# myfavouritekk/vdetlib

Hardware: AMD Instinct MI355X
Metric: boxes/sec whole-node (NMS+temporal-conv+link), 300f×10k-box synth; mAP parity (higher is better)
Workload: dtype f32; 1 GPU; configs[1]+[2]: 1 video/GPU, 300 frames x 10000 boxes x 200 classes; per-(frame,class) NMS thresh 0.30 + temporal max-pool w=3 + 3-tap temporal convolution; greedy tubelets: 10 tracks/class (stop < 0.90), IoU-link >= 0.50, spatial max-pool IoU > 0.70 + completion + temporal max-pool; frames=300, boxes=10000, classes=200, scores=rand, parallelism=video-per-gpu x1, 4 distinct videos in flight per GPU

## Files before the change

### vdetlib_amd/csrc/nms_kernels.hpp

```cpp
#pragma once
#include <hip/hip_runtime.h>
#include <stdint.h>

namespace vdet {

struct GroupDesc {
    int32_t box_off;
    int32_t nbox;
    int64_t bits_off;
};

__device__ __host__ __forceinline__ int64_t bit_word(int nbox, int v, int c)
{
    const int W = (nbox + 63) >> 6;
    return ((int64_t)(v >> 6) * W + c) * 64 + (v & 63);
}
__host__ __device__ __forceinline__ int64_t bit_words_of_group(int nbox)
{
    const int64_t W = (nbox + 63) >> 6;
    return W * W * 64;
}

struct TileDesc {
    int32_t group;
// ... 1034 lines not shown
        const uint32_t cnt = (uint32_t)__popcll(peers);
        if (act && (r1 != rank || r2 != cnt + rank)) nbad = 1;
        __builtin_amdgcn_fence(__ATOMIC_ACQ_REL, "wavefront");
    }
    if (__ballot(nbad) && lane == 0) atomicOr(bad, 1);
}

__global__ __launch_bounds__(256) void transpose_keys_kernel(const float *__restrict__ scores, uint32_t *__restrict__ keys,
                                                             int B, int C, int use_thr, float thr)
{
    __shared__ uint32_t tile[64][65];
    const int f = blockIdx.z;
    const int b0 = blockIdx.x * 64, c0 = blockIdx.y * 64;
    const int tx = threadIdx.x & 63, ty = threadIdx.x >> 6;
    const float *src = scores + (int64_t)f * B * C;
    for (int r = ty; r < 64; r += 4) {
        const int b = b0 + r, c = c0 + tx;
        uint32_t k = 0;
        if (b < B && c < C) {
            const float s = src[(int64_t)b * C + c];
            k = score_key(s);
            if (use_thr && !(s > thr)) k = 0u;
        }
        tile[r][tx] = k;
    }
    __syncthreads();
    uint32_t *dst = keys + (int64_t)f * C * B;
    for (int r = ty; r < 64; r += 4) {
        const int c = c0 + r, b = b0 + tx;
        if (c < C && b < B) dst[(int64_t)c * B + b] = tile[tx][r];
    }
}

struct WalkParams {
    int mode, P, B, C;
    const GroupDesc *groups;
    const uint16_t *order;
    const int32_t *ncand;
    const uint2 *row_meta;
    const uint16_t *adj;
    const uint32_t *group_z;
    int32_t *keep_idx;
    int32_t *keep_cnt;
    int64_t cap;
    int *status;
    int mask_words;
    const uint32_t *group_flags;
    int wave_words;
    int packed;
    const WalkMeta *wmeta;
    float t32;
    int adj32;
    const uint4 *wmeta16;
};

typedef __attribute__((address_space(3))) uint32_t lds_u32_t;
typedef volatile lds_u32_t *lds_mask_t;

__device__ __forceinline__ lds_mask_t lds_mask_ptr(unsigned char *dyn_smem, int word_off)
{
    return (lds_mask_t)((__attribute__((address_space(3))) unsigned char *)dyn_smem) + word_off;
}
__device__ __forceinline__ void lds_or(lds_mask_t m, int word, uint32_t bits)
{
    __hip_atomic_fetch_or((lds_u32_t *)(m + word), bits, __ATOMIC_RELAXED, __HIP_MEMORY_SCOPE_WAVEFRONT);
}
__device__ __forceinline__ void lds_and(lds_mask_t m, int word, uint32_t bits)
{
    __hip_atomic_fetch_and((lds_u32_t *)(m + word), bits, __ATOMIC_RELAXED, __HIP_MEMORY_SCOPE_WAVEFRONT);
}

__device__ __forceinline__ void lds_or_pair(lds_mask_t m, uint32_t d)
{
    uint32_t w0, w1;
    asm("v_bfe_u32 %0, %1, 5, 11" : "=v"(w0) : "v"(d));
    asm("v_bfe_u32 %0, %1, 21, 11" : "=v"(w1) : "v"(d));
    lds_or(m, (int)w0, 1u << (d & 31u));
    lds_or(m, (int)w1, 1u << ((d >> 16) & 31u));
}

constexpr int kWalkGrp = 4;

template <bool HASZ>
__device__ __forceinline__ void walk_apply_slice(lds_mask_t mask, uint16_t e, bool in_range, int &bad)
{
    if (HASZ) {
        if (in_range) {
            const int v = e & 0x7FFF;
            if (e & kZTag) { if (!((mask[v >> 5] >> (v & 31)) & 1u)) bad = 1; }
            else lds_or(mask, v >> 5, 1u << (v & 31));
        }
    } else {
        if (in_range) lds_or(mask, e >> 5, 1u << (e & 31));
    }
}

template <bool HASZ>
__device__ __forceinline__ void walk_group(lds_mask_t mask, const uint16_t *__restrict__ adj, int lane, int c,
                                           uint32_t off, int deg, const int (&ls)[kWalkGrp], int ng,
                                           const uint32_t (&pre)[kWalkGrp], unsigned long long &kept_lanes, int &bad)
{
#pragma unroll
    for (int k = 0; k < kWalkGrp; ++k) {
        if (k >= ng) break;
        const int cu = __builtin_amdgcn_readlane(c, ls[k]);
        if (__builtin_amdgcn_readfirstlane((mask[cu >> 5] >> (cu & 31)) & 1u)) continue;
// ... 56 lines not shown
        if (surv_s) {
            const int pos = nk + (int)__builtin_amdgcn_mbcnt_hi((uint32_t)(surv_s >> 32),
                                                               __builtin_amdgcn_mbcnt_lo((uint32_t)surv_s, 0u));
            if (surv && sub == 0 && (int64_t)pos < cap) out[(uint32_t)pos] = cm;
            nk += __popcll(surv_s);
            const uint32_t off = surv ? __float_as_uint(mi.y) : 0u;
            const int deg = surv ? (int)__float_as_uint(mi.z) : 0;
            AdjVec a0, a1;
            if (prm.adj32) {
                const uint32_t bo = off * 2u;
                const char *ab = reinterpret_cast<const char *>(prm.adj);
                a0 = *reinterpret_cast<const AdjVec *>(ab + (bo + (8 * sub < deg ? 16u * (uint32_t)sub : 0u)));
                a1 = *reinterpret_cast<const AdjVec *>(ab + (bo + (64 + 8 * sub < deg ? 128u + 16u * (uint32_t)sub : 0u)));
            } else {
                const AdjVec *pa = reinterpret_cast<const AdjVec *>(prm.adj + off);
                a0 = pa[8 * sub < deg ? sub : 0];
                a1 = pa[64 + 8 * sub < deg ? 8 + sub : 0];
            }
            const bool has0 = 8 * sub < deg, has1 = 64 + 8 * sub < deg;
            if (has0) {
#pragma unroll
                for (int t = 0; t < 4; ++t) {
                    const uint32_t d = a0.v[t];
                    lds_or_pair(mask, d);
                }
            }
            if (__ballot(has1) != 0ull) {
                if (has1) {
#pragma unroll
                    for (int t = 0; t < 4; ++t) {
                        const uint32_t d = a1.v[t];
                        lds_or_pair(mask, d);
                    }
                }
                unsigned long long lg = __ballot(sub == 0 && deg > 128);
                while (lg) {
                    const int l = __ffsll((unsigned long long)lg) - 1;
                    lg &= lg - 1;
                    const uint32_t o = __builtin_amdgcn_readlane(off, l);
                    const int dl = __builtin_amdgcn_readlane(deg, l);
                    for (int e0 = 128; e0 < dl; e0 += 64) {
                        const uint32_t e = prm.adj[o + min(e0 + lane, dl - 1)];
                        if (e0 + lane < dl) lds_or(mask, (int)(e >> 5), 1u << (e & 31u));
                    }
                }
            }
            __builtin_amdgcn_s_waitcnt(0x0F70);
        }
        qh = ring_wrap(qh + ng);
        qn -= ng;
    }
}

template <bool U16>
__device__ __forceinline__ void walk_list_packed(const WalkParams &prm, lds_mask_t mask, const int lane, const int rb,
                                                 const uint16_t *__restrict__ order, const int ncand,
                                                 int32_t *__restrict__ out, const int64_t cap, int &nk_out)
{
    lds_mask_t ring = mask + prm.mask_words;
    lds_f4_t ringb = (lds_f4_t)ring;
    const WalkMeta *__restrict__ wmeta = prm.wmeta + rb;
    const uint4 *__restrict__ wm16 = U16 ? prm.wmeta16 + rb : nullptr;
    const float t32 = prm.t32;
    int qh = 0, qn = 0, nk = 0;
    const int last = max(ncand - 1, 0);
    int cc[3];
    uint2 mm[3];
    float4 bb[3];
    uint4 rr[3];
    cc[0] = (int)order[(uint32_t)min(lane, last)];
    cc[1] = (int)order[(uint32_t)min(64 + lane, last)];
    cc[2] = 0;
    mm[0] = mm[1] = mm[2] = make_uint2(0u, 0u);
    bb[0] = bb[1] = bb[2] = make_float4(0.f, 0.f, 0.f, 0.f);
    rr[0] = rr[1] = rr[2] = make_uint4(0u, 0u, 0u, 0u);
    if (lane < ncand) {
        if (U16) rr[0] = wm16[(uint32_t)cc[0]];
        else { const WalkMeta *wm = wmeta + (uint32_t)cc[0]; bb[0] = wm->box; const uint4 rw = wm->row; mm[0] = make_uint2(rw.x, rw.y); }
    }
#define VDET_WALK_PASS(Q0, CUR, NXT, NN)                                                                                             \
    {                                                                                                                                \
        const int q0_ = (Q0);                                                                                                        \
        const int c = cc[CUR];                                                                                                       \
        cc[NN] = (int)order[(uint32_t)min(q0_ + 128 + lane, last)];                                                                  \
        {    \
             \
            const bool want = (q0_ + 64 + lane) < ncand && !((mask[cc[NXT] >> 5] >> (cc[NXT] & 31)) & 1u);                           \
            if (U16) rr[NXT] = wm16[want ? (uint32_t)cc[NXT] : 0u];                                                                  \
            else {                                                                                                                   \
                const WalkMeta *wm = wmeta + (want ? (uint32_t)cc[NXT] : 0u);                                                        \
                bb[NXT] = wm->box; const uint4 rw = wm->row; mm[NXT] = make_uint2(rw.x, rw.y);                                       \
            }                                                                                                                        \
        }                                                                                                                            \
        const bool alive = (q0_ + lane) < ncand && !((mask[c >> 5] >> (c & 31)) & 1u);                                               \
        const unsigned long long am = __ballot(alive);                                                                               \
        if (alive) {                                                                                                                 \
            const int s = ring_wrap(qh + qn + (int)__builtin_amdgcn_mbcnt_hi((uint32_t)(am >> 32), __builtin_amdgcn_mbcnt_lo((uint32_t)am, 0u))); \
            ring[8 * s] = (uint32_t)c;                                                                                               \
            lds_f4v bv;                                                                                                              \
            if (U16) {                                                                                                               \
                ring[8 * s + 1] = rr[CUR].z;                                                                                         \
                ring[8 * s + 2] = rr[CUR].w;                                                                                         \
                bv.x = (float)(rr[CUR].x & 0xFFFFu); bv.y = (float)(rr[CUR].x >> 16);                                                \
                bv.z = (float)(rr[CUR].y & 0xFFFFu); bv.w = (float)(rr[CUR].y >> 16);                                                \
            } else {                                                                                                                 \
                ring[8 * s + 1] = mm[CUR].x;                                                                                         \
                ring[8 * s + 2] = mm[CUR].y;                                                                                         \
                bv.x = bb[CUR].x; bv.y = bb[CUR].y; bv.z = bb[CUR].z; bv.w = bb[CUR].w;                                              \
            }                                                                                                                        \
            ringb[2 * s + 1] = bv;                                                                                                   \
            ring[8 * s + 3] = __float_as_uint(box_area(make_float4(bv.x, bv.y, bv.z, bv.w)));                                        \
        }                                                                                                                            \
        qn += __popcll(am);                                                                                                          \
        walk_ring_drain(prm, mask, ring, ringb, lane, t32, q0_ + 64 >= ncand, qh, qn, nk, out, cap);                                 \
    }
    for (int q0 = 0; q0 < ncand; q0 += 192) {
        VDET_WALK_PASS(q0, 0, 1, 2)
        if (q0 + 64 >= ncand) break;
        VDET_WALK_PASS(q0 + 64, 1, 2, 0)
        if (q0 + 128 >= ncand) break;
        VDET_WALK_PASS(q0 + 128, 2, 0, 1)
    }
#undef VDET_WALK_PASS
    nk_out = nk;
}

__device__ __forceinline__ void walk_one(const WalkParams &prm, const int p, unsigned char *smem, const int lane, const int w)
{
    lds_mask_t mask = lds_mask_ptr(smem, w * prm.wave_words);
    const ProblemRef pr = decode_problem(prm.mode, p, prm.B, prm.C, prm.groups);
    const int N = pr.N, rb = pr.rb;
    const uint16_t *order = prm.order + pr.obase;
    const int ncand = prm.ncand[p];
    const bool has_z = prm.group_z[pr.g] != 0;
    const bool regular = !has_z && prm.group_flags && (prm.group_flags[pr.g] & kFlagRegular);
    int32_t *out = prm.keep_idx + (prm.mode == 2 ? (int64_t)rb : (int64_t)p * prm.cap);
    const int64_t cap = prm.mode == 2 ? (int64_t)N : prm.cap;

    for (int i = lane; i < ((N + 31) >> 5); i += 64) mask[i] = 0u;
    __builtin_amdgcn_fence(__ATOMIC_ACQ_REL, "wavefront");
    if (has_z) {
        for (int q = ncand + lane; q < N; q += 64) {
            const int v = order[q];
            lds_or(mask, v >> 5, 1u << (v & 31));
        }
        __builtin_amdgcn_fence(__ATOMIC_ACQ_REL, "wavefront");
    }

    int nk = 0;
    int bad = 0;
    if (regular && prm.packed && N >= 2) {
        if (prm.wmeta16 && (prm.group_flags[pr.g] & kFlagU16)) walk_list_packed<true>(prm, mask, lane, rb, order, ncand, out, cap, nk);
        else walk_list_packed<false>(prm, mask, lane, rb, order, ncand, out, cap, nk);
        if (lane == 0) prm.keep_cnt[p] = nk;
        if ((int64_t)nk > cap && lane == 0) atomicOr(prm.status, kStCap);
        return;
    }
    const uint32_t *adjw = reinterpret_cast<const uint32_t *>(prm.adj);
    const int last = max(ncand - 1, 0);
    int c_cur = (int)order[min(lane, last)];
    int c_nxt = (int)order[min(64 + lane, last)];
    uint2 m_cur = make_uint2(0u, 0u);
    if (lane < ncand) m_cur = prm.row_meta[rb + c_cur];
    for (int q0 = 0; q0 < ncand; q0 += 64) {
        const int q = q0 + lane;
        const bool valid = q < ncand;
        const int c = c_cur;
        const int c_nn = (int)order[min(q0 + 128 + lane, last)];
        uint2 m_nxt = make_uint2(0u, 0u);
        if ((q + 64) < ncand && !((mask[c_nxt >> 5] >> (c_nxt & 31)) & 1u)) m_nxt = prm.row_meta[rb + c_nxt];
        const bool alive = valid && !((mask[c >> 5] >> (c & 31)) & 1u);
        unsigned long long am = __ballot(alive);
        unsigned long long kept_lanes = 0ull;
        const uint32_t off = m_cur.x;
        const int deg = (int)m_cur.y;
        while (am) {
            int ls[kWalkGrp];
            int ng = 0;
#pragma unroll
            for (int k = 0; k < kWalkGrp; ++k) {
                ls[k] = k ? ls[k - 1] : 0;
                if (am) { ls[k] = __builtin_amdgcn_readfirstlane(__ffsll((unsigned long long)am) - 1); am &= am - 1; ng = k + 1; }
            }
            uint32_t pre[kWalkGrp];
#pragma unroll
            for (int k = 0; k < kWalkGrp; ++k) {
                const uint32_t o = __builtin_amdgcn_readlane(off, ls[k]);
                const int d = __builtin_amdgcn_readlane(deg, ls[k]);
                pre[k] = adjw[(o >> 1) + min(lane, (max(d, 1) - 1) >> 1)];
            }
            if (has_z) walk_group<true>(mask, prm.adj, lane, c, off, deg, ls, ng, pre, kept_lanes, bad);
            else walk_group<false>(mask, prm.adj, lane, c, off, deg, ls, ng, pre, kept_lanes, bad);
        }
        if (kept_lanes) {
            const int pos = nk + (int)__builtin_amdgcn_mbcnt_hi((uint32_t)(kept_lanes >> 32),
                                                               __builtin_amdgcn_mbcnt_lo((uint32_t)kept_lanes, 0u));
            if (((kept_lanes >> lane) & 1ull) && (int64_t)pos < cap) out[pos] = c;
            nk += __popcll(kept_lanes);
        }
        c_cur = c_nxt; c_nxt = c_nn; m_cur = m_nxt;
    }
    if (lane == 0) prm.keep_cnt[p] = nk;
    if ((int64_t)nk > cap && lane == 0) atomicOr(prm.status, kStCap);
    if (__ballot(bad != 0) && lane == 0) atomicOr(prm.status, kStDivZero);
}

__global__ __launch_bounds__(256) void walk_kernel(const WalkParams prm)
{
    extern __shared__ __attribute__((aligned(16))) unsigned char smem[];
    const int lane = threadIdx.x & 63, w = __builtin_amdgcn_readfirstlane(threadIdx.x >> 6);
    const int nwaves_total = gridDim.x * 4;
    const int per = nwaves_total >> 3;
    const int p = (blockIdx.x & 7) * per + (blockIdx.x >> 3) * 4 + w;
    if (p >= prm.P) return;
    walk_one(prm, p, smem, lane, w);
}

__global__ __launch_bounds__(256) void check_order_kernel(const uint16_t *__restrict__ order, const int32_t *__restrict__ ncand_in, int P, int B,
                                                          int32_t *__restrict__ ncand_out, int *__restrict__ status)
{
    const int lane = threadIdx.x & 63;
    const int p = blockIdx.x * 4 + (threadIdx.x >> 6);
    if (p >= P) return;
    const int n = ncand_in[p];
    bool bad = n < 0 || n > B;
    if (!bad)
        for (int q = lane; q < n; q += 64) bad = bad || (int)order[(int64_t)p * B + q] >= B;
    const bool any = __ballot(bad) != 0ull;
    if (lane == 0) {
        ncand_out[p] = any ? 0 : n;
        if (any) atomicOr(status, kStBadOrder);
    }
}

__global__ __launch_bounds__(256) void gather_comp_kernel(const GroupDesc *__restrict__ groups, int P,
                                                          const int32_t *__restrict__ keep_idx,
                                                          const int32_t *__restrict__ keep_cnt,
                                                          const float *__restrict__ scores,
                                                          const uint32_t *__restrict__ keys,
                                                          const uint32_t *__restrict__ orig_idx,
                                                          unsigned long long *__restrict__ comp,
                                                          unsigned int *__restrict__ glob_cnt)
{
    __shared__ unsigned int sbase;
    const int p = blockIdx.x;
    if (p >= P) return;
    const int rb = groups[p].box_off;
    const int K = keep_cnt[p];
    if (threadIdx.x == 0) sbase = atomicAdd(glob_cnt, (unsigned int)K);
    __syncthreads();
    const unsigned int base = sbase;
    for (int k = threadIdx.x; k < K; k += 256) {
        const int v = keep_idx[rb + k];
        const uint32_t key = keys ? keys[rb + v] : score_key(scores[rb + v]);
        comp[base + k] = ((unsigned long long)key << 32) | orig_idx[rb + v];
    }
}

__global__ void bitonic_global_step(unsigned long long *__restrict__ data, uint32_t n2, uint32_t j, uint32_t k)
{
// ... 95 lines not shown
```

### vdetlib_amd/csrc/vdet_capi.hip

```cpp
#include <hip/hip_runtime.h>
#include <atomic>
#include <chrono>

#include <algorithm>
#include <cmath>
#include <cstdarg>
#include <cstdio>
#include <cstdlib>
#include <cstring>
#include <initializer_list>
#include <string>
#include <vector>

#include "../../include/vdet_hip.h"
#include "nms_kernels.hpp"
#include "binsort_kernels.hpp"
#include "small_kernels.hpp"
#include "detnms_kernels.hpp"
#include "fused_kernels.hpp"
#include "adjrows_kernels.hpp"
#include "graphlists_kernels.hpp"
#include "temporal_kernels.hpp"
#include "tubelet_kernels.hpp"
#include "track_kernels.hpp"
// ... 108 lines not shown
    int n_cu = 256;
    DevBuf boxes, scores, keys, excl, frames, groups, tiles, bits, rowz, rowmeta, groupz, adj, comp, origidx,
        out64, trk_frames, trk_boxes, b1, b2, iou_out, order, ncand, keepidx, keepcnt, gflags, pairs, tkeys, tstate, visited, heads, xkeys, xord, wmeta, wmeta16, reachtab, rowperm, qreach, ditems, striptot, stripoff, xncand, xbox, xbox16, xord16, xcum, xinfo, tmp[8];
    bool timing = false;
    bool timing_accumulate = false;
    std::vector<std::pair<hipEvent_t, hipEvent_t>> ev_pool;
    std::vector<int> ev_stage;
    size_t ev_used = 0;
    float last_ms[ST_COUNT] = {0};
    int last_launches[ST_COUNT] = {0};
    bool sort_attr_set = false;
    bool cache_enabled = false;
    struct PrepKey { const void *boxes = nullptr; int64_t F = 0, B = 0; float t32 = 0; ListsKey lists; } prep;
    bool graph_valid = false, lists_valid = false;
    struct KeySrc { const void *scores = nullptr; int64_t F = 0, B = 0, C = 0; int use_thr = 0; float thr = 0; } keysrc;
    bool keys_valid = false;
    bool vpass_attr_set = false;
    int vpass_form = VDET_VPASS_AUTO;
    int vpass_fchunk = 0;
    int vpass_last_items = 0;
    bool index_valid = false; const void *index_boxes = nullptr; int64_t index_F = 0, index_B = 0;
    bool all_regular = false;
    bool wave_transpose = false;
    bool no_lazy = false;
    bool no_index = false;
    bool force_general = false;
    bool atomic_rank = false;
    bool small_lists = true;
    bool adj_rows = true;
    bool direct_lists = true;
    uint32_t direct_cap = 384;
    int64_t direct_ntot = 0;
    unsigned long long direct_fixed = 0;
    bool no_fused = false;
    bool binsort = true;
    bool binsort_inherit = true;
    int binsort_grid = 0;
    const std::vector<GroupDesc> *host_groups = nullptr;
    bool sym_built = false;
    NmsPlan vplan;
    bool vplan_valid = false;
    int64_t vplan_F = 0, vplan_B = 0;
    size_t vplan_budget = 0;
    long long n_host_syncs = 0;
    bool async_enabled = false;
    unsigned long long pool_hint = 0;
    bool topk_attr_set = false;
    float gt32 = 0.f;
    bool wmeta16_built = false;
    bool wmeta_built = false;
    bool last_sort_binned = false;
    StagedTab vidtab, segtab;
    DevBuf sortctl;
    DevBuf nover;
    DevBuf ordncand;
    DevBuf linkmemo, linkstats, linkwarm, linkorder, linkchains, linknodes, tracknode, rtodo;
    struct NodeKey { const void *tracks = nullptr, *boxes = nullptr; int64_t F = 0, B = 0, C = 0; int T = 0; double nms_thres = 0; } nodekey;
    bool nodes_valid = false;
    void *fused_in = nullptr, *fused_out = nullptr;
    void *fused_in_dev = nullptr, *fused_out_dev = nullptr;
    void *fbatch_in = nullptr, *fbatch_out = nullptr, *fbatch_in_dev = nullptr, *fbatch_out_dev = nullptr;
    size_t fbatch_in_cap = 0, fbatch_out_cap = 0;
    bool fbatch_attr = false;
    size_t dyn_lds_max = 0;
    DevBuf ev_tab, ev_dtp, ev_dsc, ev_dslot, ev_bcnt, ev_boff, ev_key[2], ev_val[2], ev_hist;
    DevBuf tcn_x, tcn_frames, tcn_base, tcn_len, tcn_scratch, tcn_h0;
    StagedTab tcn_params, tcn_foff, tcn_ovtab, tcn_segs;
    bool tcn_tiled = false;
    bool tcn_global = false;
    StagedTab interp_tab;
    StagedTab anchor_tab;
    DevBuf topa_hist, topa_state, topa_cnt, topa_nrec, topa_rec;
    bool topa_hist_clean = false;
    DevBuf svm_wt, svm_wavebad;
    StagedTab ctxs_tab;
    DevBuf ctxs_hist, ctxs_state, ctxs_rec;
    int64_t ctxs_last_videos = 0;
    bool ctxs_records = true;
    DevBuf sq_link, sq_live, sq_done, sq_ptr;
    bool sq_lds = true;
    bool sq_attr_set = false;
    int sq_last_path = -1;
};

namespace {

hipError_t host_sync(vdet_ctx *c)
{
    ++c->n_host_syncs;
    return hipStreamSynchronize(c->stream);
}

int fail(vdet_ctx *c, int code, const char *fmt, ...)
{
    char buf[512];
    va_list ap;
    va_start(ap, fmt);
    vsnprintf(buf, sizeof buf, fmt, ap);
    va_end(ap);
    if (c) c->err = buf;
    return code;
}

#define HIPCHK(c, expr)                                                                          \
    do {                                                                                         \
        hipError_t _e = (expr);                                                                  \
// ... 720 lines not shown
            HIPCHK(c, hipLaunchKernel(fn, dim3(grid), dim3(256), args, 0, c->stream));
        } else if (use_bin) {
            HIPCHK(c, c->sortctl.reserve(sizeof(BinSortCtl) + (size_t)a.P * 4));
            HIPCHK(c, hipMemsetAsync(c->sortctl.p, 0, sizeof(BinSortCtl), c->stream));
            BinSortParams bp{};
            const bool floats = sp.keys == nullptr;
            bp.raw = floats ? reinterpret_cast<const uint32_t *>(sp.scores) : sp.keys;
            bp.P = a.P; bp.N = a.B;
            bp.order = sp.order; bp.ncand = sp.ncand;
            bp.ctl = c->sortctl.as<BinSortCtl>();
            bp.fail_list = reinterpret_cast<int32_t *>(c->sortctl.as<char>() + sizeof(BinSortCtl));
            const int per_cu = std::max<int>(1, (int)(c->max_lds / (bin_lds + 4096)));
            bp.inherit = c->binsort_inherit ? 1 : 0;
            const int full = std::min(a.P, per_cu * c->n_cu);
            const int grid = c->binsort_grid > 0 ? std::min(full, c->binsort_grid) : full;
#define VDET_BSK(CP) (floats ? reinterpret_cast<const void *>(binsort_kernel<CP, true>) : reinterpret_cast<const void *>(binsort_kernel<CP, false>))
            const void *bfn = bin_cpw == 8 ? VDET_BSK(8) : bin_cpw == 20 ? VDET_BSK(20) : VDET_BSK(36);
#undef VDET_BSK
            void *bargs[] = {&bp};
            HIPCHK(c, hipLaunchKernel(bfn, dim3(grid), dim3(512), bargs, bin_lds, c->stream));
            const int32_t *fl = bp.fail_list;
            const int *fc = &bp.ctl->nfail;
            void *largs[] = {&sp, (void *)&fl, (void *)&fc};
            StageTimer tm2(c, ST_SORTFB);
            HIPCHK(c, hipLaunchKernel(var->fn_list[c->atomic_rank ? 1 : 0], dim3(std::min(a.P, 2 * c->n_cu)), dim3(block), largs, lds, c->stream));
        } else {
            const int grid = (a.P + 7) & ~7;
            void *args[] = {&sp};
            HIPCHK(c, hipLaunchKernel(var->fn[c->atomic_rank ? 1 : 0], dim3(grid), dim3(block), args, lds, c->stream));
        }
    }
    HIPCHK(c, hipGetLastError());
    if (a.sort_only) return VDET_OK;
    WalkParams wp{};
    wp.mode = a.mode; wp.P = a.P; wp.B = a.B; wp.C = a.C;
    wp.groups = c->groups.as<GroupDesc>();
    wp.order = a.order_in ? a.order_in : c->order.as<uint16_t>();
    wp.ncand = a.order_in ? a.ncand_in : c->ncand.as<int32_t>();
    wp.row_meta = c->rowmeta.as<uint2>();
    wp.adj = c->adj.as<uint16_t>();
    wp.group_z = c->groupz.as<uint32_t>();
    wp.keep_idx = a.keep_idx;
    wp.keep_cnt = a.keep_cnt;
    wp.cap = a.cap;
    wp.status = &c->d_cnt->status;
    wp.mask_words = (int)(r16((size_t)4 * ((std::max(nmax, 1) + 31) / 32)) / 4);
    wp.group_flags = c->sym_built ? c->gflags.as<uint32_t>() : nullptr;
    wp.packed = (wp.group_flags && c->wmeta_built) ? 1 : 0;
    wp.wave_words = wp.mask_words + (wp.packed ? 8 * kPackRing : 0);
    wp.wmeta = c->wmeta.as<WalkMeta>();
    wp.t32 = c->gt32;
    wp.wmeta16 = (wp.packed && c->wmeta16_built) ? c->wmeta16.as<uint4>() : nullptr;
    wp.adj32 = c->adj.cap <= 0xFFFFFF00ull ? 1 : 0;
    const bool small_walk = c->small_lists && a.mode != 2 && nmax <= kSmallMax && wp.group_flags && a.C > 0 && a.P % a.C == 0;
    if (small_walk) {
        const int G = a.P / a.C;
        const int nq = nmax <= 128 ? 1 : nmax <= 256 ? 2 : 3;
        const int nm = std::max(nmax, 1);
        const size_t row_bytes = (size_t)nm * 4 * nq * 4;
        const int fpw = a.C > 32 ? 1 : (int)std::max<size_t>(1, std::min<size_t>((size_t)(64 / a.C), (size_t)(44 * 1024) / row_bytes));
        const size_t lds_bytes = (size_t)fpw * row_bytes;
        const int vec4 = (a.B % 4 == 0 && ((uintptr_t)wp.order & 7) == 0) ? 1 : 0;
        const int grid = (G + fpw - 1) / fpw;
        StageTimer tm(c, ST_WALK);
#define VDET_SMALLW(NQ_, V_) hipLaunchKernelGGL((small_walk_kernel<NQ_, V_>), dim3(grid), dim3(64), lds_bytes, c->stream, wp, G, fpw, nm)
        if (vec4) { if (nq == 1) VDET_SMALLW(1, true); else if (nq == 2) VDET_SMALLW(2, true); else VDET_SMALLW(3, true); }
        else { if (nq == 1) VDET_SMALLW(1, false); else if (nq == 2) VDET_SMALLW(2, false); else VDET_SMALLW(3, false); }
#undef VDET_SMALLW
        if (!c->all_regular)
            hipLaunchKernelGGL(walk_rest_kernel, dim3(std::min(G, 4 * c->n_cu)), dim3(256), (size_t)wp.wave_words * 4 * 4, c->stream, wp, G);
    } else {
        const int nblk = (((a.P + 3) / 4) + 7) & ~7;
        StageTimer tm(c, ST_WALK);
        hipLaunchKernelGGL(walk_kernel, dim3(nblk), dim3(256), (size_t)wp.wave_words * 4 * 4, c->stream, wp);
    }
    HIPCHK(c, hipGetLastError());
    return VDET_OK;
}

int volume_lists(vdet_ctx *c, const float *d_boxes, const float *d_scores, int64_t F, int64_t B, int64_t C, double nms_thres, bool reuse)
{
    bool same_geo = false;
    const int rc = ensure_volume_graph(c, d_boxes, F, B, nms_thres, reuse, &same_geo);
    if (rc || (same_geo && lists_match(c, ListsKey{d_scores, C, VDET_LAYOUT_FBC, 0, 0.f, 0}, F, B))) return rc;
    return launch_sort_walk(c, volume_sort_args(F, B, C, d_scores), (int)B, F * C * B);
}

int track_begin(vdet_ctx *c, int64_t C, int max_tracks, int32_t *d_ntracks)
{
    c->lists_valid = false;
    hipLaunchKernelGGL(track_init_kernel, dim3((unsigned)((C + 63) / 64)), dim3(64), 0, c->stream, c->tstate.as<TrackState>(), (int)C);
    HIPCHK(c, hipMemsetAsync(d_ntracks, 0, (size_t)C * 4, c->stream));
    if (max_tracks == 0) HIPCHK(c, hipGetLastError());
    return VDET_OK;
}

struct GreedyArgs { SuppressParams sp; LazyLists lz; LoopArgs la; };

GreedyArgs greedy_args(vdet_ctx *c, const TrackWork &w, const float *d_boxes, const float *d_scores, int64_t F, int64_t B, int64_t C,
                       double nms_thres, double thres, int max_tracks, float *d_tracks, float *d_anchors, int32_t *d_ntracks)
{
    GreedyArgs g{};
    SuppressParams &sp = g.sp;
    sp.boxes = reinterpret_cast<const float4 *>(d_boxes);
    sp.F = (int)F; sp.B = (int)B; sp.C = (int)C; sp.max_tracks = max_tracks;
    sp.groups = c->groups.as<GroupDesc>();
// ... 301 lines not shown
        for (int64_t q = 0; q < nk; ++q) h_keep[h_off[k] + q] = kept[h_off[k] + q];
    }
    if (divz) return fail(c, VDET_EDIVZERO, "float division (zero union)");
    return VDET_OK;
}

}

extern "C" {

const char *vdet_version(void) { return "vdet_hip 0.1 gfx950"; }

int vdet_create(vdet_ctx **out, int device)
{
    if (!out) return VDET_EINVAL;
    *out = nullptr;
    vdet_ctx *c = new (std::nothrow) vdet_ctx;
    if (!c) return VDET_ENOMEM;
    int ndev = 0;
    if (hipGetDeviceCount(&ndev) != hipSuccess || ndev <= 0) {
        delete c;
        return VDET_EHIP;
    }
    if (device < 0) {
        if (hipGetDevice(&device) != hipSuccess) { delete c; return VDET_EHIP; }
    }
    if (device >= ndev || hipSetDevice(device) != hipSuccess) { delete c; return VDET_EINVAL; }
    c->device = device;
    hipDeviceProp_t prop;
    if (hipGetDeviceProperties(&prop, device) == hipSuccess) {
        c->n_cu = prop.multiProcessorCount > 0 ? prop.multiProcessorCount : 256;
        if (strncmp(prop.gcnArchName, "gfx950", 6) != 0) c->max_lds = 64 * 1024;
    }
    if (const char *e = getenv("VDET_FORCE_GENERAL")) c->force_general = atoi(e) != 0;
    if (const char *e = getenv("VDET_BITS_BUDGET_MB")) {
        const long mb = atol(e);
        if (mb > 0) c->bits_budget = (size_t)mb << 20;
    }
    if (hipStreamCreateWithFlags(&c->own_stream, hipStreamNonBlocking) != hipSuccess ||
        hipMalloc((void **)&c->d_cnt, sizeof(Counters)) != hipSuccess) {
        delete c;
        return VDET_EHIP;
    }
    c->stream = c->own_stream;
    (void)hipMemsetAsync(c->d_cnt, 0, sizeof(Counters), c->stream);
    if (const char *e = getenv("VDET_NO_INDEX")) c->no_index = atoi(e) != 0;
    if (const char *e = getenv("VDET_NO_LAZY")) c->no_lazy = atoi(e) != 0;
    if (const char *e = getenv("VDET_NO_FUSED")) c->no_fused = atoi(e) != 0;
    if (const char *e = getenv("VDET_ADJ_ROWS")) c->adj_rows = atoi(e) != 0;
    if (const char *e = getenv("VDET_DIRECT_LISTS")) c->direct_lists = atoi(e) != 0;
    if (const char *e = getenv("VDET_DIRECT_CAP")) { const int v = atoi(e); if (v >= 8 && v <= 32760) c->direct_cap = (uint32_t)(v & ~7); }
    if (const char *e = getenv("VDET_BINSORT")) c->binsort = atoi(e) != 0;
    if (const char *e = getenv("VDET_BINSORT_INHERIT")) c->binsort_inherit = atoi(e) != 0;
    if (const char *e = getenv("VDET_BINSORT_GRID")) { const int v = atoi(e); if (v >= 1) c->binsort_grid = v; }
    if (const char *e = getenv("VDET_SMALL_LISTS")) c->small_lists = atoi(e) != 0;
    if (const char *e = getenv("VDET_TCN_TILED")) c->tcn_tiled = atoi(e) != 0;
    if (const char *e = getenv("VDET_TCN_GLOBAL")) c->tcn_global = atoi(e) != 0;
    if (const char *e = getenv("VDET_CTX_RECORDS")) c->ctxs_records = atoi(e) != 0;
    if (const char *e = getenv("VDET_SEQNMS_LDS")) c->sq_lds = atoi(e) != 0;
    if (const char *e = getenv("VDET_VPASS_FORM")) { const int v = atoi(e); if (v >= VDET_VPASS_AUTO && v <= VDET_VPASS_ONE_PER_CU) c->vpass_form = v; }
    if (const char *e = getenv("VDET_VPASS_FCHUNK")) { const int v = atoi(e); if (v >= 1) c->vpass_fchunk = v; }
    {
        const int npat = 4096;
        std::vector<uint8_t> pats((size_t)npat * 64);
        uint32_t rs = 12345u;
        auto rnd = [&]() { rs = rs * 1664525u + 1013904223u; return rs >> 8; };
        for (int t = 0; t < npat; ++t) {
            const int kind = t % 8;
            const int nd = kind == 0 ? 1 : kind == 1 ? 2 : kind == 2 ? 3 : kind == 3 ? 8 : kind == 4 ? 32 : kind == 5 ? 64 : kind == 6 ? 200 : 254;
            for (int l = 0; l < 64; ++l) {
                uint8_t d = (uint8_t)(rnd() % nd);
                if (kind == 7 && (rnd() & 3) == 0) d = 255;
                if (t % 16 == 9) d = (uint8_t)((l * (1 + t % 7)) % nd);
                pats[(size_t)t * 64 + l] = d;
            }
        }
        bool ok = false;
        DevBuf pb;
        if (pb.reserve(pats.size()) == hipSuccess &&
            hipMemcpyAsync(pb.p, pats.data(), pats.size(), hipMemcpyHostToDevice, c->stream) == hipSuccess) {
            hipLaunchKernelGGL(lds_atomic_order_probe, dim3(256), dim3(64), 0, c->stream, pb.as<uint8_t>(), npat,
                               &c->d_cnt->status);
            Counters h;
            if (hipMemcpyAsync(&h, c->d_cnt, sizeof h, hipMemcpyDeviceToHost, c->stream) == hipSuccess &&
                host_sync(c) == hipSuccess)
                ok = (h.status == 0);
        }
        pb.release();
        (void)hipMemsetAsync(c->d_cnt, 0, sizeof(Counters), c->stream);
        c->atomic_rank = ok;
        if (const char *e = getenv("VDET_ATOMIC_RANK")) c->atomic_rank = c->atomic_rank && atoi(e) != 0;
    }
    {
        const int n = 64;
        std::vector<uint64_t> hin((size_t)n * 64), hout((size_t)n * 64);
        uint64_t x = 0x9E3779B97F4A7C15ull;
        for (size_t i = 0; i < hin.size(); ++i) {
            x ^= x << 13; x ^= x >> 7; x ^= x << 17;
            hin[i] = (i / 64) == 0 ? (1ull << (i % 64)) : ((i / 64) == 1 ? (uint64_t)(i % 64 == 5 ? ~0ull : 0ull) : x);
        }
        bool ok = false;
        DevBuf bi, bo;
        if (bi.reserve(hin.size() * 8) == hipSuccess && bo.reserve(hin.size() * 8) == hipSuccess &&
            hipMemcpyAsync(bi.p, hin.data(), hin.size() * 8, hipMemcpyHostToDevice, c->stream) == hipSuccess) {
            hipLaunchKernelGGL(wave_transpose_probe, dim3(16), dim3(64), 0, c->stream, bi.as<uint64_t>(), bo.as<uint64_t>(), n);
            if (hipMemcpyAsync(hout.data(), bo.p, hout.size() * 8, hipMemcpyDeviceToHost, c->stream) == hipSuccess &&
                host_sync(c) == hipSuccess) {
                ok = true;
                for (int t = 0; t < n && ok; ++t)
                    for (int r = 0; r < 64 && ok; ++r)
                        for (int k = 0; k < 64; ++k)
                            if (((hin[(size_t)t * 64 + r] >> k) & 1ull) != ((hout[(size_t)t * 64 + k] >> r) & 1ull)) { ok = false; break; }
            }
        }
        bi.release(); bo.release();
        c->wave_transpose = ok;
        if (const char *e = getenv("VDET_WAVE_TRANSPOSE")) c->wave_transpose = c->wave_transpose && atoi(e) != 0;
    }
    *out = c;
    return VDET_OK;
}

int vdet_destroy(vdet_ctx *c)
{
    if (!c) return VDET_OK;
    (void)hipSetDevice(c->device);
    (void)host_sync(c);
    DevBuf *bufs[] = {&c->boxes, &c->scores, &c->keys, &c->excl, &c->frames, &c->groups, &c->tiles, &c->bits,
                      &c->rowz, &c->rowmeta, &c->groupz, &c->adj, &c->comp, &c->origidx, &c->out64,
                      &c->trk_frames, &c->trk_boxes, &c->b1, &c->b2, &c->iou_out, &c->order, &c->ncand, &c->keepidx,
                      &c->keepcnt, &c->gflags, &c->pairs, &c->tkeys, &c->tstate, &c->visited, &c->heads, &c->xkeys, &c->xord, &c->xncand, &c->linkmemo, &c->linkstats, &c->linkwarm, &c->linkorder, &c->linkchains, &c->linknodes, &c->tracknode, &c->rtodo,
                      &c->xbox, &c->xbox16, &c->xord16, &c->xcum, &c->xinfo, &c->wmeta, &c->wmeta16, &c->reachtab, &c->rowperm, &c->qreach, &c->ditems, &c->striptot, &c->stripoff, &c->sortctl, &c->segtab.dev, &c->vidtab.dev, &c->nover, &c->ordncand, &c->ev_tab, &c->ev_dtp, &c->ev_dsc,
                      &c->ev_dslot, &c->ev_bcnt, &c->ev_boff, &c->ev_key[0], &c->ev_key[1], &c->ev_val[0], &c->ev_val[1], &c->ev_hist,
                      &c->tcn_x, &c->tcn_frames, &c->tcn_base, &c->tcn_len, &c->tcn_scratch, &c->tcn_h0, &c->tcn_params.dev, &c->tcn_foff.dev, &c->tcn_segs.dev, &c->tcn_ovtab.dev, &c->interp_tab.dev,
                      &c->anchor_tab.dev, &c->topa_hist, &c->topa_state, &c->topa_cnt, &c->topa_nrec, &c->topa_rec, &c->svm_wt, &c->svm_wavebad,
                      &c->ctxs_tab.dev, &c->ctxs_hist, &c->ctxs_state, &c->ctxs_rec, &c->sq_link, &c->sq_live, &c->sq_done, &c->sq_ptr};
    for (DevBuf *b : bufs) b->release();
    for (DevBuf &b : c->tmp) b.release();
    for (auto &e : c->ev_pool) { (void)hipEventDestroy(e.first); (void)hipEventDestroy(e.second); }
    if (c->d_cnt) (void)hipFree(c->d_cnt);
    if (c->fused_in) (void)hipHostFree(c->fused_in);
    if (c->fused_out) (void)hipHostFree(c->fused_out);
    if (c->fbatch_in) (void)hipHostFree(c->fbatch_in);
    if (c->fbatch_out) (void)hipHostFree(c->fbatch_out);
    if (c->own_stream) (void)hipStreamDestroy(c->own_stream);
    delete c;
    return VDET_OK;
}

int vdet_set_stream(vdet_ctx *c, void *s)
{
    if (!c) return VDET_EINVAL;
    c->stream = (hipStream_t)s;
    return VDET_OK;
}

int vdet_reset_stream(vdet_ctx *c)
{
    if (!c) return VDET_EINVAL;
    c->stream = c->own_stream;
    return VDET_OK;
}

const char *vdet_last_error(vdet_ctx *c) { return c ? c->err.c_str() : "null context"; }

int vdet_set_cache(vdet_ctx *c, int enable)
{
    if (!c) return VDET_EINVAL;
    c->cache_enabled = enable != 0;
    c->graph_valid = c->lists_valid = c->index_valid = c->keys_valid = c->nodes_valid = false;
    return VDET_OK;
}

int vdet_invalidate(vdet_ctx *c)
{
    if (!c) return VDET_EINVAL;
    c->graph_valid = c->lists_valid = c->index_valid = c->keys_valid = c->nodes_valid = false;
    return VDET_OK;
}

int vdet_query(vdet_ctx *c, int what)
{
    if (!c) return VDET_EINVAL;
    if (what == 0) return c->atomic_rank ? 1 : 0;
    if (what == 1) return c->n_cu;
    if (what == 2) return c->all_regular ? 1 : 0;
    if (what == 3) return c->wave_transpose ? 1 : 0;
    if (what == 15) return c->direct_ntot > 0 ? 1 : 0;
    if (what == 8) return (int)std::min<long long>(c->n_host_syncs, 0x7FFFFFFF);
    if (what == 10) return (int)std::min<long long>(c->tcn_params.uploads, 0x7FFFFFFF);
    if (what == 11) return (int)std::min<long long>(c->anchor_tab.uploads, 0x7FFFFFFF);
    if (what == 12) return c->vpass_last_items;
    if (what == 13) {
        if (c->ctxs_last_videos <= 0 || !c->ctxs_state.p) return -1;
        std::vector<CtxState> h((size_t)c->ctxs_last_videos);
        if (hipMemcpyAsync(h.data(), c->ctxs_state.p, h.size() * sizeof(CtxState), hipMemcpyDeviceToHost, c->stream) != hipSuccess ||
            host_sync(c) != hipSuccess) return VDET_EHIP;
        int reads = 0;
        for (const CtxState &st : h) reads = std::max(reads, st.empty ? 0 : 2 + (int)st.path);
        return reads;
    }
    if (what == 14) return c->sq_last_path;
    if (what == 9 || what == 16 || what == 17) {
        if (!c->last_sort_binned || !c->sortctl.p) return -1;
        BinSortCtl h{};
        if (hipMemcpyAsync(&h, c->sortctl.p, sizeof h, hipMemcpyDeviceToHost, c->stream) != hipSuccess || host_sync(c) != hipSuccess) return VDET_EHIP;
        return what == 9 ? h.nfail : what == 16 ? h.ninherit : h.nredo;
    }
    if (what >= 4 && what <= 7) {
        unsigned int h[4] = {0, 0, 0, 0};
        if (!c->linkstats.p) return 0;
        if (hipMemcpyAsync(h, c->linkstats.p, 16, hipMemcpyDeviceToHost, c->stream) != hipSuccess ||
            host_sync(c) != hipSuccess) return VDET_EHIP;
        return (int)std::min<unsigned int>(h[what - 4], 0x7FFFFFFFu);
    }
    return VDET_EINVAL;
}

int vdet_set_timing(vdet_ctx *c, int enable)
{
    if (!c) return VDET_EINVAL;
    c->timing = enable != 0;
    c->timing_accumulate = enable == 2;
    c->ev_used = 0;
    return VDET_OK;
}

int vdet_last_timing_ms(vdet_ctx *c, float *out16)
{
    float *out8 = out16;
    if (!c || !out8) return VDET_EINVAL;
    HIPCHK(c, host_sync(c));
    for (int i = 0; i < ST_COUNT; ++i) { c->last_ms[i] = 0; c->last_launches[i] = 0; }
    for (size_t i = 0; i < c->ev_used; ++i) {
        float ms = 0;
        if (hipEventElapsedTime(&ms, c->ev_pool[i].first, c->ev_pool[i].second) == hipSuccess) {
            c->last_ms[c->ev_stage[i]] += ms;
            c->last_launches[c->ev_stage[i]] += 1;
        }
    }
    for (int i = 0; i < ST_COUNT; ++i) out8[i] = c->last_ms[i];
    c->ev_used = 0;
    return VDET_OK;
}

int vdet_last_launches(vdet_ctx *c, int *out16)
{
    if (!c || !out16) return VDET_EINVAL;
    for (int i = 0; i < ST_COUNT; ++i) out16[i] = c->last_launches[i];
    return VDET_OK;
}

int vdet_sync(vdet_ctx *c)
{
    if (!c) return VDET_EINVAL;
    Counters h;
    HIPCHK(c, hipMemcpyAsync(&h, c->d_cnt, sizeof h, hipMemcpyDeviceToHost, c->stream));
    HIPCHK(c, host_sync(c));
    HIPCHK(c, hipMemsetAsync(&c->d_cnt->status, 0, kPerBuildOff, c->stream));
    h.pool_used = std::max(h.pool_used, h.pool_max);
// ... 2850 lines not shown
```

Measured before the change: 358.2 million boxes/s.

## Add wide-window greedy NMS walk that prefilters dead candidates across several batches

Once a 64-candidate pass enqueues fewer than a threshold of live boxes, the packed greedy NMS walk switches to a wide mode. It scans kWideW×64 candidates at a time, compacts the still-alive ones into an LDS stage, and double-buffers metadata loads, so far fewer mostly-dead passes are needed. If more than 64 survive, it falls back to per-64 passes. It also pins walk_kernel to 8 waves per EU, adds LDS per wave, and adds atomic stats counters plus a query API, at the cost of extra registers and LDS.

```diff
diff --git a/devtools/walk_filter_sim.py b/devtools/walk_filter_sim.py
--- /dev/null
+++ b/devtools/walk_filter_sim.py
@@ -0,0 +1,121 @@
+#!/usr/bin/env python3
+import argparse
+import os
+import sys
+
+import numpy as np
+
+sys.path.insert(0, os.path.join(os.path.dirname(os.path.dirname(os.path.abspath(__file__))), "tests"))
+import synth
+
+
+def adjacency(b, t):
+    b = b.astype(np.float64)
+    area = (b[:, 2] - b[:, 0] + 1) * (b[:, 3] - b[:, 1] + 1)
+    adj = []
+    for r0 in range(0, len(b), 1000):
+        r = b[r0:r0 + 1000]
+        w = np.minimum(r[:, None, 2], b[None, :, 2]) - np.maximum(r[:, None, 0], b[None, :, 0]) + 1
+        h = np.minimum(r[:, None, 3], b[None, :, 3]) - np.maximum(r[:, None, 1], b[None, :, 1]) + 1
+        inter = np.maximum(w, 0) * np.maximum(h, 0)
+        hit = inter >= t * (area[r0:r0 + 1000, None] + area[None, :] - inter)
+        hit[np.arange(len(r)), r0 + np.arange(len(r))] = False
+        adj.extend(np.flatnonzero(row) for row in hit)
+    return adj
+
+
+class Walk:
+    def __init__(self, adj, n):
+        self.adj, self.dead, self.ring = adj, np.zeros(n, bool), []
+        self.passes = self.groups = self.queued = self.kept = self.dead_members = self.high = self.overflow = 0
+        self.switch_at = -1
+
+    def queue(self, ids):
+        ids = [c for c in ids if not self.dead[c]]
+        self.ring.extend(ids)
+        self.queued += len(ids)
+        self.high = max(self.high, len(self.ring))
+
+    def drain(self, flush):
+        while len(self.ring) >= 8 or (flush and self.ring):
+            grp, self.ring = self.ring[:8], self.ring[8:]
+            self.groups += 1
+            live = [c for c in grp if not self.dead[c]]
+            self.dead_members += len(grp) - len(live)
+            surv = []
+            for c in live:
+                if not any(c in self.adj_set(s) for s in surv):
+                    surv.append(c)
+            for s in surv:
+                self.dead[self.adj[s]] = True
+            self.kept += len(surv)
+
+    def adj_set(self, s):
+        return set(self.adj[s].tolist())
+
+
+def walk(adj, order, W=1, nsw=-1):
+    n = len(order)
+    wk = Walk(adj, len(adj))
+    q = 0
+    while q < n:
+        before = wk.queued
+        wk.passes += 1
+        wk.queue(order[q:q + 64])
+        wk.drain(q + 64 >= n)
+        q += 64
+        if W > 1 and q > 64 and q < n and wk.queued - before <= nsw:
+            wk.switch_at = q
+            break
+    if q < n and W > 1:
+        span = 64 * W
+        want = [c for c in order[q:q + span] if not wk.dead[c]]
+        while q < n:
+            nxt = [c for c in order[q + span:q + 2 * span] if not wk.dead[c]]
+            wk.passes += 1
+            if len(want) <= 64:
+                wk.queue(want)
+                wk.drain(q + span >= n)
+            else:
+                wk.overflow += 1
+                for s in range(q, min(q + span, n), 64):
+                    wk.queue(order[s:s + 64])
+                    wk.drain(s + 64 >= n)
+            q += span
+            want = nxt
+    return wk
+
+
+def main():
+    ap = argparse.ArgumentParser()
+    ap.add_argument("--boxes", type=int, default=10000)
+    ap.add_argument("--thresh", type=float, default=0.3)
+    ap.add_argument("--orders", type=int, default=3)
+    ap.add_argument("--canvas", type=float, default=1.0, help="shrink the recipe's canvas (denser frames)")
+    ap.add_argument("--seed", type=int, default=2000)
+    a = ap.parse_args()
+    rng = np.random.RandomState(a.seed)
+    b = synth.boxes_1(rng, a.boxes)
+    if a.canvas != 1.0:
+        b[:, [0, 2]] *= a.canvas
+        b[:, [1, 3]] *= a.canvas
+        b = np.round(b)
+    adj = adjacency(b, a.thresh)
+    print("boxes %d  threshold %.2f  average degree %.1f" % (a.boxes, a.thresh, np.mean([len(x) for x in adj])))
+    rules = [("today", 1, -1)] + [("W=%d nsw=%d" % (W, nsw), W, nsw) for W in (4, 8) for nsw in (8, 12, 16, 24)]
+    print("%-14s %5s %6s %6s %6s %6s %5s %5s %7s %5s" % ("rule", "order", "passes", "groups", "queued", "kept", "dead", "ring", "switch", "ovfl"))
+    ref = None
+    for name, W, nsw in rules:
+        for o in range(a.orders):
+            order = np.random.RandomState(a.seed + 1 + o).permutation(a.boxes)
+            wk = walk(adj, order, W, nsw)
+            if W == 1:
+                ref = ref or {}
+                ref[o] = wk.kept
+            assert wk.kept == ref[o], "the wide rule changed the result"
+            print("%-14s %5d %6d %6d %6d %6d %5d %5d %7d %5d" % (name, o, wk.passes, wk.groups, wk.queued, wk.kept, wk.dead_members, wk.high,
+                                                                   wk.switch_at, wk.overflow))
+
+
+if __name__ == "__main__":
+    main()
diff --git a/vdetlib_amd/csrc/nms_kernels.hpp b/vdetlib_amd/csrc/nms_kernels.hpp
--- a/vdetlib_amd/csrc/nms_kernels.hpp
+++ b/vdetlib_amd/csrc/nms_kernels.hpp
@@ -1110,6 +1110,8 @@
     float t32;
     int adj32;
     const uint4 *wmeta16;
+    int wide_nsw;
+    uint32_t *wide_stats;
 };
 
 typedef __attribute__((address_space(3))) uint32_t lds_u32_t;
@@ -1272,10 +1274,51 @@
     }
 }
 
+#ifndef VDET_WALK_W
+#define VDET_WALK_W 4
+#endif
+constexpr int kWideW = VDET_WALK_W;
+constexpr int kWideSpan = 64 * kWideW;
+constexpr int kWideStage = 64;
+constexpr int kWideStatSlots = 64;
+
+template <bool U16>
+__device__ __forceinline__ void walk_rec_load(const WalkMeta *__restrict__ wmeta, const uint4 *__restrict__ wm16, const uint32_t id,
+                                              uint4 &r, float4 &b, uint2 &m)
+{
+    if (U16) r = wm16[id];
+    else { const WalkMeta *wm = wmeta + id; b = wm->box; const uint4 rw = wm->row; m = make_uint2(rw.x, rw.y); }
+}
+
+template <bool U16>
+__device__ __forceinline__ void walk_ring_push(lds_mask_t ring, lds_f4_t ringb, const int qh, int &qn, const bool alive, const int c,
+                                               const uint4 &r, const float4 &b, const uint2 &m)
+{
+    const unsigned long long am = __ballot(alive);
+    if (alive) {
+        const int s = ring_wrap(qh + qn + (int)__builtin_amdgcn_mbcnt_hi((uint32_t)(am >> 32), __builtin_amdgcn_mbcnt_lo((uint32_t)am, 0u)));
+        ring[8 * s] = (uint32_t)c;
+        lds_f4v bv;
+        if (U16) {
+            ring[8 * s + 1] = r.z;
+            ring[8 * s + 2] = r.w;
+            bv.x = (float)(r.x & 0xFFFFu); bv.y = (float)(r.x >> 16);
+            bv.z = (float)(r.y & 0xFFFFu); bv.w = (float)(r.y >> 16);
+        } else {
+            ring[8 * s + 1] = m.x;
+            ring[8 * s + 2] = m.y;
+            bv.x = b.x; bv.y = b.y; bv.z = b.z; bv.w = b.w;
+        }
+        ringb[2 * s + 1] = bv;
+        ring[8 * s + 3] = __float_as_uint(box_area(make_float4(bv.x, bv.y, bv.z, bv.w)));
+    }
+    qn += __popcll(am);
+}
+
 template <bool U16>
 __device__ __forceinline__ void walk_list_packed(const WalkParams &prm, lds_mask_t mask, const int lane, const int rb,
                                                  const uint16_t *__restrict__ order, const int ncand,
-                                                 int32_t *__restrict__ out, const int64_t cap, int &nk_out)
+                                                 int32_t *__restrict__ out, const int64_t cap, int &nk_out, int &wide_in, int &wide_ovf)
 {
     lds_mask_t ring = mask + prm.mask_words;
     lds_f4_t ringb = (lds_f4_t)ring;
@@ -1331,17 +1374,89 @@
             ringb[2 * s + 1] = bv;                                                                                                   \
             ring[8 * s + 3] = __float_as_uint(box_area(make_float4(bv.x, bv.y, bv.z, bv.w)));                                        \
         }                                                                                                                            \
-        qn += __popcll(am);                                                                                                          \
+        nq_last = __popcll(am);                                                                                                      \
+        qn += nq_last;                                                                                                               \
         walk_ring_drain(prm, mask, ring, ringb, lane, t32, q0_ + 64 >= ncand, qh, qn, nk, out, cap);                                 \
     }
+    const int nsw = prm.wide_nsw;
+    int nq_last = 0, qw = ncand;
     for (int q0 = 0; q0 < ncand; q0 += 192) {
         VDET_WALK_PASS(q0, 0, 1, 2)
         if (q0 + 64 >= ncand) break;
+        if (nq_last < nsw) { qw = q0 + 64; break; }
         VDET_WALK_PASS(q0 + 64, 1, 2, 0)
         if (q0 + 128 >= ncand) break;
+        if (nq_last < nsw) { qw = q0 + 128; break; }
         VDET_WALK_PASS(q0 + 128, 2, 0, 1)
+        if (q0 + 192 < ncand && nq_last < nsw) { qw = q0 + 192; break; }
     }
 #undef VDET_WALK_PASS
+    if (qw < ncand) wide_in = 1;
+    while (qw < ncand) {
+        lds_mask_t stage = ring + 8 * kPackRing;
+        int id0[kWideW], id1[kWideW];
+        int c0 = 0, c1 = 0, n0 = 0, n1 = 0;
+        uint4 r0 = make_uint4(0u, 0u, 0u, 0u), r1 = r0;
+        float4 b0 = make_float4(0.f, 0.f, 0.f, 0.f), b1 = b0;
+        uint2 m0 = make_uint2(0u, 0u), m1 = m0;
+#define VDET_WIDE_IDS(QB, ID)                                                                                                        \
+        _Pragma("unroll") for (int j = 0; j < kWideW; ++j) ID[j] = (int)order[(uint32_t)min((QB) + 64 * j + lane, last)];
+#define VDET_WIDE_STAGE1(QB, ID, CC, NC, R, BX, M)                                                                                   \
+        {                                                                                                                            \
+            uint32_t mw[kWideW];                                                                                                     \
+            _Pragma("unroll") for (int j = 0; j < kWideW; ++j) mw[j] = mask[ID[j] >> 5];                                              \
+            int tot = 0;                                                                                                             \
+            _Pragma("unroll") for (int j = 0; j < kWideW; ++j) {                                                                     \
+                const bool want = ((QB) + 64 * j + lane) < ncand && !((mw[j] >> (ID[j] & 31)) & 1u);                                 \
+                const unsigned long long wm = __ballot(want);                                                                        \
+                const int at = tot + (int)__builtin_amdgcn_mbcnt_hi((uint32_t)(wm >> 32), __builtin_amdgcn_mbcnt_lo((uint32_t)wm, 0u)); \
+                if (want && at < kWideStage) stage[at] = (uint32_t)ID[j];                                                            \
+                tot += __popcll(wm);                                                                                                 \
+            }                                                                                                                        \
+            NC = tot;                                                                                                                \
+            const uint32_t sid = stage[lane];                                                                                        \
+            CC = lane < tot ? (int)sid : 0;                                                                                          \
+            walk_rec_load<U16>(wmeta, wm16, (uint32_t)CC, R, BX, M);                                                                 \
+        }
+#define VDET_WIDE_STAGE2(QB, CC, NC, R, BX, M)                                                                                       \
+        {                                                                                                                            \
+            const uint32_t mc = mask[CC >> 5];                                                                                       \
+            const bool alive = lane < NC && !((mc >> (CC & 31)) & 1u);                                                               \
+            walk_ring_push<U16>(ring, ringb, qh, qn, alive, CC, R, BX, M);                                                           \
+            walk_ring_drain(prm, mask, ring, ringb, lane, t32, (QB) + kWideSpan >= ncand, qh, qn, nk, out, cap);                     \
+        }
+        VDET_WIDE_IDS(qw, id0)
+        VDET_WIDE_IDS(qw + kWideSpan, id1)
+        VDET_WIDE_STAGE1(qw, id0, c0, n0, r0, b0, m0)
+        bool over = false;
+        for (;; qw += 2 * kWideSpan) {
+            VDET_WIDE_IDS(qw + 2 * kWideSpan, id0)
+            VDET_WIDE_STAGE1(qw + kWideSpan, id1, c1, n1, r1, b1, m1)
+            if (n0 > kWideStage) { over = true; break; }
+            VDET_WIDE_STAGE2(qw, c0, n0, r0, b0, m0)
+            if (qw + kWideSpan >= ncand) { qw = ncand; break; }
+            VDET_WIDE_IDS(qw + 3 * kWideSpan, id1)
+            VDET_WIDE_STAGE1(qw + 2 * kWideSpan, id0, c0, n0, r0, b0, m0)
+            if (n1 > kWideStage) { over = true; qw += kWideSpan; break; }
+            VDET_WIDE_STAGE2(qw + kWideSpan, c1, n1, r1, b1, m1)
+            if (qw + 2 * kWideSpan >= ncand) { qw = ncand; break; }
+        }
+#undef VDET_WIDE_IDS
+#undef VDET_WIDE_STAGE1
+#undef VDET_WIDE_STAGE2
+        if (!over) break;
+        ++wide_ovf;
+        const int qe = min(qw + kWideSpan, ncand);
+        for (int qs = qw; qs < qe; qs += 64) {
+            const int id = (int)order[(uint32_t)min(qs + lane, last)];
+            const bool alive = (qs + lane) < ncand && !((mask[id >> 5] >> (id & 31)) & 1u);
+            uint4 rs = make_uint4(0u, 0u, 0u, 0u); float4 bs = make_float4(0.f, 0.f, 0.f, 0.f); uint2 ms = make_uint2(0u, 0u);
+            walk_rec_load<U16>(wmeta, wm16, alive ? (uint32_t)id : 0u, rs, bs, ms);
+            walk_ring_push<U16>(ring, ringb, qh, qn, alive, id, rs, bs, ms);
+            walk_ring_drain(prm, mask, ring, ringb, lane, t32, qs + 64 >= ncand, qh, qn, nk, out, cap);
+        }
+        qw = qe;
+    }
     nk_out = nk;
 }
 
@@ -1370,8 +1485,13 @@
     int nk = 0;
     int bad = 0;
     if (regular && prm.packed && N >= 2) {
-        if (prm.wmeta16 && (prm.group_flags[pr.g] & kFlagU16)) walk_list_packed<true>(prm, mask, lane, rb, order, ncand, out, cap, nk);
-        else walk_list_packed<false>(prm, mask, lane, rb, order, ncand, out, cap, nk);
+        int wide_in = 0, wide_ovf = 0;
+        if (prm.wmeta16 && (prm.group_flags[pr.g] & kFlagU16)) walk_list_packed<true>(prm, mask, lane, rb, order, ncand, out, cap, nk, wide_in, wide_ovf);
+        else walk_list_packed<false>(prm, mask, lane, rb, order, ncand, out, cap, nk, wide_in, wide_ovf);
+        if (wide_in && lane == 0) {
+            atomicAdd(prm.wide_stats + (p & (kWideStatSlots - 1)), 1u);
+            if (wide_ovf) atomicAdd(prm.wide_stats + kWideStatSlots + (p & (kWideStatSlots - 1)), (uint32_t)wide_ovf);
+        }
         if (lane == 0) prm.keep_cnt[p] = nk;
         if ((int64_t)nk > cap && lane == 0) atomicOr(prm.status, kStCap);
         return;
@@ -1425,7 +1545,7 @@
     if (__ballot(bad != 0) && lane == 0) atomicOr(prm.status, kStDivZero);
 }
 
-__global__ __launch_bounds__(256) void walk_kernel(const WalkParams prm)
+__global__ __launch_bounds__(256) __attribute__((amdgpu_waves_per_eu(8, 8))) void walk_kernel(const WalkParams prm)
 {
     extern __shared__ __attribute__((aligned(16))) unsigned char smem[];
     const int lane = threadIdx.x & 63, w = __builtin_amdgcn_readfirstlane(threadIdx.x >> 6);
diff --git a/vdetlib_amd/csrc/vdet_capi.hip b/vdetlib_amd/csrc/vdet_capi.hip
--- a/vdetlib_amd/csrc/vdet_capi.hip
+++ b/vdetlib_amd/csrc/vdet_capi.hip
@@ -184,6 +184,9 @@
     bool last_sort_binned = false;
     StagedTab vidtab, segtab;
     DevBuf sortctl;
+    int walk_wide_nsw = 12;
+    bool last_walk_wide = false;
+    DevBuf walkstats;
     DevBuf nover;
     DevBuf ordncand;
     DevBuf linkmemo, linkstats, linkwarm, linkorder, linkchains, linknodes, tracknode, rtodo;
@@ -1010,6 +1013,14 @@
     wp.t32 = c->gt32;
     wp.wmeta16 = (wp.packed && c->wmeta16_built) ? c->wmeta16.as<uint4>() : nullptr;
     wp.adj32 = c->adj.cap <= 0xFFFFFF00ull ? 1 : 0;
+    wp.wide_nsw = wp.packed ? c->walk_wide_nsw : 0;
+    if (wp.packed) wp.wave_words += kWideStage;
+    c->last_walk_wide = wp.wide_nsw > 0;
+    if (wp.wide_nsw > 0) {
+        HIPCHK(c, c->walkstats.reserve(sizeof(uint32_t) * 2 * kWideStatSlots));
+        HIPCHK(c, hipMemsetAsync(c->walkstats.p, 0, sizeof(uint32_t) * 2 * kWideStatSlots, c->stream));
+        wp.wide_stats = c->walkstats.as<uint32_t>();
+    }
     const bool small_walk = c->small_lists && a.mode != 2 && nmax <= kSmallMax && wp.group_flags && a.C > 0 && a.P % a.C == 0;
     if (small_walk) {
         const int G = a.P / a.C;
@@ -1417,6 +1428,8 @@
     if (const char *e = getenv("VDET_DIRECT_CAP")) { const int v = atoi(e); if (v >= 8 && v <= 32760) c->direct_cap = (uint32_t)(v & ~7); }
     if (const char *e = getenv("VDET_BINSORT")) c->binsort = atoi(e) != 0;
     if (const char *e = getenv("VDET_BINSORT_INHERIT")) c->binsort_inherit = atoi(e) != 0;
+    if (const char *e = getenv("VDET_WALK_WIDE")) { if (atoi(e) == 0) c->walk_wide_nsw = 0; }
+    if (const char *e = getenv("VDET_WALK_WIDE_NSW")) { const int v = atoi(e); if (v >= 1 && v <= 63 && c->walk_wide_nsw > 0) c->walk_wide_nsw = v; }
     if (const char *e = getenv("VDET_BINSORT_GRID")) { const int v = atoi(e); if (v >= 1) c->binsort_grid = v; }
     if (const char *e = getenv("VDET_SMALL_LISTS")) c->small_lists = atoi(e) != 0;
     if (const char *e = getenv("VDET_TCN_TILED")) c->tcn_tiled = atoi(e) != 0;
@@ -1495,7 +1508,7 @@
                       &c->rowz, &c->rowmeta, &c->groupz, &c->adj, &c->comp, &c->origidx, &c->out64,
                       &c->trk_frames, &c->trk_boxes, &c->b1, &c->b2, &c->iou_out, &c->order, &c->ncand, &c->keepidx,
                       &c->keepcnt, &c->gflags, &c->pairs, &c->tkeys, &c->tstate, &c->visited, &c->heads, &c->xkeys, &c->xord, &c->xncand, &c->linkmemo, &c->linkstats, &c->linkwarm, &c->linkorder, &c->linkchains, &c->linknodes, &c->tracknode, &c->rtodo,
-                      &c->xbox, &c->xbox16, &c->xord16, &c->xcum, &c->xinfo, &c->wmeta, &c->wmeta16, &c->reachtab, &c->rowperm, &c->qreach, &c->ditems, &c->striptot, &c->stripoff, &c->sortctl, &c->segtab.dev, &c->vidtab.dev, &c->nover, &c->ordncand, &c->ev_tab, &c->ev_dtp, &c->ev_dsc,
+                      &c->xbox, &c->xbox16, &c->xord16, &c->xcum, &c->xinfo, &c->wmeta, &c->wmeta16, &c->reachtab, &c->rowperm, &c->qreach, &c->ditems, &c->striptot, &c->stripoff, &c->sortctl, &c->walkstats, &c->segtab.dev, &c->vidtab.dev, &c->nover, &c->ordncand, &c->ev_tab, &c->ev_dtp, &c->ev_dsc,
                       &c->ev_dslot, &c->ev_bcnt, &c->ev_boff, &c->ev_key[0], &c->ev_key[1], &c->ev_val[0], &c->ev_val[1], &c->ev_hist,
                       &c->tcn_x, &c->tcn_frames, &c->tcn_base, &c->tcn_len, &c->tcn_scratch, &c->tcn_h0, &c->tcn_params.dev, &c->tcn_foff.dev, &c->tcn_segs.dev, &c->tcn_ovtab.dev, &c->interp_tab.dev,
                       &c->anchor_tab.dev, &c->topa_hist, &c->topa_state, &c->topa_cnt, &c->topa_nrec, &c->topa_rec, &c->svm_wt, &c->svm_wavebad,
@@ -1571,6 +1584,14 @@
         BinSortCtl h{};
         if (hipMemcpyAsync(&h, c->sortctl.p, sizeof h, hipMemcpyDeviceToHost, c->stream) != hipSuccess || host_sync(c) != hipSuccess) return VDET_EHIP;
         return what == 9 ? h.nfail : what == 16 ? h.ninherit : h.nredo;
+    }
+    if (what == 18 || what == 19) {
+        if (!c->last_walk_wide || !c->walkstats.p) return -1;
+        uint32_t h[2 * kWideStatSlots];
+        if (hipMemcpyAsync(h, c->walkstats.p, sizeof h, hipMemcpyDeviceToHost, c->stream) != hipSuccess || host_sync(c) != hipSuccess) return VDET_EHIP;
+        unsigned long long n = 0;
+        for (int i = 0; i < kWideStatSlots; ++i) n += h[(what - 18) * kWideStatSlots + i];
+        return (int)std::min<unsigned long long>(n, 0x7FFFFFFFull);
     }
     if (what >= 4 && what <= 7) {
         unsigned int h[4] = {0, 0, 0, 0};
```

Result: faster. 367.8 million boxes/s (median of 6 runs) (+2.7%).
